# feihoo87/waveforms

Measured on AMD Instinct MI355X. Metric: Msamples/s (all channels), higher is better.
Workload: dtype f64; 1 GPU; sampler256: 256 ch/GPU x 1e+07 pts, 100 gaussian+DRAG pulses/ch, seeds 1000+c (SURVEY 8(d) C4/C5 channel spec), grid mode; channels_per_gpu=256, channels_total=256, points_per_channel=10000000, output=device (HBM) buffer, parallelism=channel-block-per-rank x1, no data-path collective

## Files before the change

### waveforms_amd/csrc/wfk_chain_dev.h

```cpp
#pragma once
#include <hip/hip_runtime.h>

#include <type_traits>
#include <utility>

#include "wfk_internal.h"

namespace {

template <int... K, typename F>
__device__ __forceinline__ void sfor_impl(std::integer_sequence<int, K...>, F&& f) {
  (f(std::integral_constant<int, K>{}), ...);
}
template <int N, typename F>
__device__ __forceinline__ void sfor(F&& f) {
  sfor_impl(std::make_integer_sequence<int, N>{}, static_cast<F&&>(f));
}
#define CH_EACH(N, k) sfor<N>([&](auto k##_) __attribute__((always_inline)) { constexpr int k = decltype(k##_)::value;
#define CH_END });

__device__ __forceinline__ int cuni(int v) { return __builtin_amdgcn_readfirstlane(v); }
__device__ __forceinline__ int64_t cuni64(int64_t v) {
  return (int64_t)(((uint64_t)(uint32_t)cuni((int)(v >> 32)) << 32) | (uint32_t)cuni((int)v));
}

struct ChSeeds { double c, s, g, r; };

__device__ __forceinline__ double kc(double v) {
  asm volatile("" : "+s"(v));
  return v;
}

__device__ __forceinline__ void sincospi_small(double r, double* sn, double* cs) {
  const double a = fabs(r);
  const bool swap = a > 0.25;
  const double z = swap ? 0.5 - a : a;
  const double t = z * 3.141592653589793116 + z * 1.2246467991473532e-16;
  const double t2 = t * t;
  double ps = kc(-2.8114572543455206e-15);
  ps = fma(ps, t2, kc(7.6471637318198164e-13));
  ps = fma(ps, t2, kc(-1.6059043836821613e-10));
  ps = fma(ps, t2, kc(2.5052108385441720e-08));
  ps = fma(ps, t2, kc(-2.7557319223985893e-06));
  ps = fma(ps, t2, kc(1.9841269841269841e-04));
  ps = fma(ps, t2, kc(-8.3333333333333332e-03));
  ps = fma(ps, t2, kc(1.6666666666666666e-01));
  const double s = fma(-t * t2, ps, t);
  double pc = kc(1.5619206968586226e-16);
  pc = fma(pc, t2, kc(-4.7794773323873853e-14));
  pc = fma(pc, t2, kc(1.1470745597729725e-11));
  pc = fma(pc, t2, kc(-2.0876756987868099e-09));
  pc = fma(pc, t2, kc(2.7557319223985888e-07));
  pc = fma(pc, t2, kc(-2.4801587301587302e-05));
  pc = fma(pc, t2, kc(1.3888888888888889e-03));
  pc = fma(pc, t2, kc(-4.1666666666666664e-02));
  pc = fma(pc, t2, kc(0.5));
  const double c = fma(-t2, pc, 1.0);
  const double ss = swap ? c : s, cc = swap ? s : c;
  *sn = r < 0.0 ? -ss : ss;
  *cs = cc;
}

__device__ __forceinline__ double exp_small(double x) {
#pragma clang fp contract(off)
  const double n = rint(x * 1.4426950408889634);
  double r = fma(-n, 6.93147180369123816490e-01, x);
  r = fma(-n, 1.90821492927058770002e-10, r);
  double p = kc(1.1470745597729725e-11);
  p = fma(p, r, kc(1.6059043836821613e-10));
  p = fma(p, r, kc(2.0876756987868099e-09));
  p = fma(p, r, kc(2.5052108385441720e-08));
  p = fma(p, r, kc(2.7557319223985888e-07));
  p = fma(p, r, kc(2.7557319223985893e-06));
  p = fma(p, r, kc(2.4801587301587302e-05));
  p = fma(p, r, kc(1.9841269841269841e-04));
  p = fma(p, r, kc(1.3888888888888889e-03));
  p = fma(p, r, kc(8.3333333333333332e-03));
  p = fma(p, r, kc(4.1666666666666664e-02));
  p = fma(p, r, kc(1.6666666666666666e-01));
  p = fma(p, r, kc(0.5));
  p = fma(p, r, kc(1.0));
  p = fma(p, r, kc(1.0));
  return ldexp(p, (int)n);
}

__device__ __forceinline__ ChSeeds chain_seeds(double theta, double ea, double eb, int carrier, int env) {
#pragma clang fp contract(off)
  ChSeeds o;
  o.c = 1.0; o.s = 0.0; o.g = 1.0; o.r = 1.0;
  if (carrier) {
    const double IPI_HI = 0.31830988618379069, IPI_LO = -1.9678676675182486e-17;
    const double xh = theta * IPI_HI;
    const double xl = fma(theta, IPI_HI, -xh) + theta * IPI_LO;
    const double n = rint(xh);
    double ss, cc;
    sincospi_small((xh - n) + xl, &ss, &cc);
    const bool odd = ((long long)n) & 1;
    o.s = odd ? -ss : ss;
    o.c = odd ? -cc : cc;
  }
  if (env) {
    o.g = exp_small(ea);
    o.r = exp_small(eb);
  }
  return o;
}

template <typename T, int CL, int KC, bool MASK, bool DEG1, bool SEL = false, bool INIT = false>
__device__ __forceinline__ void chain_loop(const double2* tab, const double* r, const ChSeeds& sd, double u0,
                                           double q, T (&acc)[CL], int klo, int khi, ChSeeds& nx) {
  const T c0 = (T)sd.c, s0 = (T)sd.s;
  const T A0 = (T)r[WFK_FCE_A], A1 = (T)r[WFK_FCE_A + 1], A2 = (T)r[WFK_FCE_A + 2], A3 = (T)r[WFK_FCE_A + 3];
  const T B0 = (T)r[WFK_FCE_B], B1 = (T)r[WFK_FCE_B + 1], B2 = (T)r[WFK_FCE_B + 2], B3 = (T)r[WFK_FCE_B + 3];
  const T P0 = DEG1 ? A0 * c0 + B0 * s0 : (T)0, P1 = DEG1 ? A1 * c0 + B1 * s0 : (T)0;
  const T Q0 = DEG1 ? B0 * c0 - A0 * s0 : (T)0, Q1 = DEG1 ? B1 * c0 - A1 * s0 : (T)0;
  double g = sd.g, rr = sd.r;
  T u = (T)u0;
  const T Dt = (T)r[WFK_FCE_D];
#ifndef WFK_FIRS_SB
#define WFK_FIRS_SB 1
#endif
  constexpr int SB = CL % WFK_FIRS_SB == 0 ? WFK_FIRS_SB : 2;
  static_assert(CL % SB == 0, "chain length must be even");
  CH_EACH(CL / SB, kb)
    double2 tb[SB];
    CH_EACH(SB, kk) tb[kk] = tab[kb * SB + kk]; CH_END
    CH_EACH(SB, kk)
      constexpr int k = kb * SB + kk;
      T val;
      if constexpr (DEG1) {
        const T pp = P1 * u + P0, qq = Q1 * u + Q0;
        u += Dt;
        val = (pp * (T)tb[kk].x + qq * (T)tb[kk].y) * (T)g;
      } else {
        const T pa = ((A3 * u + A2) * u + A1) * u + A0;
        const T pb = ((B3 * u + B2) * u + B1) * u + B0;
        u += Dt;
        const T ck = c0 * (T)tb[kk].x - s0 * (T)tb[kk].y;
        const T sk = s0 * (T)tb[kk].x + c0 * (T)tb[kk].y;
        val = (pa * ck + pb * sk) * (T)g;
      }
      if constexpr (k == KC) {
        nx.g = g;
        nx.r = rr;
        nx.c = sd.c * tb[kk].x - sd.s * tb[kk].y;
        nx.s = sd.s * tb[kk].x + sd.c * tb[kk].y;
      }
      g *= rr;
      rr *= q;
      if constexpr (INIT) acc[k] = val;
      else if constexpr (MASK && SEL) acc[k] += (k >= klo && k < khi) ? val : (T)0;
      else if (!MASK || (k >= klo && k < khi)) acc[k] += val;
    CH_END
    __builtin_amdgcn_sched_barrier(0);
  CH_END
  if constexpr (KC == CL) {
    const double2 te = tab[CL];
    nx.g = g;
    nx.r = rr;
    nx.c = sd.c * te.x - sd.s * te.y;
    nx.s = sd.s * te.x + sd.c * te.y;
  }
}

__device__ __forceinline__ ChSeeds chain_make_seeds(const double* r, double x, int fl) {
  const double v = (x - r[WFK_FCE_SG]) / r[WFK_FCE_SIGMA], Hh = r[WFK_FCE_H];
  if (fl & WFK_FCE_EXPENV)
    return chain_seeds(r[WFK_FCE_W] * (x - r[WFK_FCE_SREF]), r[WFK_FCE_SIGMA] * (x - r[WFK_FCE_SG]), Hh,
                       (fl >> 2) & 1, true);
  return chain_seeds(r[WFK_FCE_W] * (x - r[WFK_FCE_SREF]), -(v * v), -Hh * (2.0 * v + Hh), (fl >> 2) & 1,
                     ((fl >> 4) & 3) != 0);
}

template <typename T, int CL, int KC, bool SEL = false>
__device__ __forceinline__ void chain_envmul(const double* r, const ChSeeds& sd, T (&acc)[CL], int klo, int khi,
                                             ChSeeds& nx) {
  double g = sd.g, rr = sd.r;
  const double q = r[WFK_FCE_Q];
  nx = sd;
  CH_EACH(CL, k)
    if constexpr (k == KC) {
      nx.g = g;
      nx.r = rr;
    }
    if constexpr (SEL) acc[k] *= (k >= klo && k < khi) ? (T)g : (T)1;
    else if (k >= klo && k < khi) acc[k] *= (T)g;
    g *= rr;
    rr *= q;
  CH_END
  if constexpr (KC == CL) {
    nx.g = g;
    nx.r = rr;
  }
}

}
```

### waveforms_amd/csrc/wfk_fir_sampled.hip

```cpp
#include <hip/hip_runtime.h>

#include <algorithm>
#include <cmath>
#include <cstring>
#include <memory>
#include <new>
#include <string>
#include <type_traits>
#include <utility>
#include <vector>

#include "wfk.h"
#include "wfk_fft4096.h"
#include "wfk_host.h"
#include "wfk_internal.h"
#include "wfk_short_dev.h"
#include "wfk_chain_dev.h"

namespace {

struct ChainArgs {
  const DevChannel* channels;
  const DevPiece* pieces;
  const double* params;
  const int32_t* pair_first;
  void* out;
  int64_t out_stride, n, npairs;
  const void* hspec;
  const void* tw;
  double t0, step, last;
  int32_t has_last, hop, K, lead;
  int64_t hrow;
  int64_t i0;
};

__device__ __forceinline__ double chain_time(const ChainArgs& a, int64_t j) {
#pragma clang fp contract(off)
  const double m = (double)(j + a.i0) * a.step;
  double t = m + a.t0;
  if (a.has_last && j == a.n - 1) t = a.last;
  return t;
}

#ifndef WFK_FIRS_WAVES
#define WFK_FIRS_WAVES 3
#endif
#ifndef WFK_FIRS_PPW
#define WFK_FIRS_PPW 1
#endif
#define WFK_FIRS_NCAR 2

template <typename T, int HOPB>
__global__ void __launch_bounds__(256, WFK_FIRS_WAVES) fir_sampled(const ChainArgs a) {
  constexpr int CL = 16 + HOPB;
  constexpr int PPW = WFK_FIRS_PPW, NCAR = WFK_FIRS_NCAR;
  constexpr bool CARRY = PPW > 1;
  constexpr int KC = CARRY ? 2 * HOPB : -1;
  static_assert(KC < CL, "the chains of consecutive pairs must overlap");
  __shared__ __attribute__((aligned(16))) T lds[LDS_ELEMS];
  double* const s_par = reinterpret_cast<double*>(lds);
  constexpr int LDS_DOUBLES = (int)(sizeof(T) * LDS_ELEMS / sizeof(double));
  double2* const unit_tab = reinterpret_cast<double2*>(s_par + LDS_DOUBLES - 2 * CL);
  const int tid = threadIdx.x;
  const int ch = blockIdx.y;
  const DevChannel C = a.channels[ch];
  const cx<T>* hspec = static_cast<const cx<T>*>(a.hspec) + (int64_t)ch * a.hrow;
  const cx<T>* tw = static_cast<const cx<T>*>(a.tw);
  T* const orow = static_cast<T*>(a.out) + (int64_t)ch * a.out_stride;
  const int M = a.hop;

  int car_piece = -1;
  ChSeeds car[NCAR];
  for (int i = 0; i < NCAR; ++i) { car[i].c = 1.0; car[i].s = 0.0; car[i].g = 1.0; car[i].r = 1.0; }

  for (int pp = 0; pp < PPW; ++pp) {
    const int64_t pair = (int64_t)blockIdx.x * PPW + pp;
    if (pair >= a.npairs) break;
    const int64_t s1 = 2 * pair * (int64_t)a.hop - a.lead;
    const int64_t range_end = s1 + 256 * (int64_t)CL;

    T acc[CL];
    CH_EACH(CL, k) acc[k] = (T)0; CH_END
    double x = chain_time(a, s1 + tid);
    if (C.tshift != 0.0) x = x - C.tshift;
    __syncthreads();
    if (tid < CL) unit_tab[tid] = make_double2(1.0, 0.0);
    int next_car = -1;
    int q = cuni(a.pair_first[(int64_t)ch * a.npairs + pair]);
    for (; q < C.piece_end; q = cuni(q + 1)) {
      const DevPiece P = a.pieces[q];
      if (P.start >= range_end) break;
      if (P.n_blk == 0 || P.stop <= s1) continue;
      __syncthreads();
      for (int i = tid; i < P.first_len; i += 256) s_par[i] = a.params[P.par_off + i];
      __syncthreads();
      const int nops = cuni((int)s_par[1]);
      const bool full = P.start <= s1 && P.stop >= range_end;
      const bool carried = CARRY && full && car_piece == q;
      int klo = 0, khi = CL;
      if (!full) {
        const int64_t lim = 256 * (int64_t)(CL + 2);
        const int64_t los = P.start - s1, his = P.stop - s1;
        const int lo = (int)(los < -lim ? -lim : (los > lim ? lim : los)) - tid;
        const int hi = (int)(his < -lim ? -lim : (his > lim ? lim : his)) - tid;
        klo = lo <= 0 ? 0 : (lo + 255) >> 8;
        khi = hi <= 0 ? 0 : (hi + 255) >> 8;
        klo = klo > CL ? CL : klo;
        khi = khi > CL ? CL : khi;
      }
      for (int op = 0; op < nops; ++op) {
        const double* rec = s_par + WFK_BLK_HDR + op * WFK_FCE_REC;
        const int fl = cuni(WFK_FCE_WORD(rec));
        const int env = (fl >> 4) & 3, carrier = (fl >> 2) & 1;
        ChSeeds sd, nx;
        if (carried && op == 0) sd = car[0];
        else if (carried && NCAR > 1 && op == 1) sd = car[NCAR > 1 ? 1 : 0];
        else sd = chain_make_seeds(rec, x, fl);
        if (env == 3) {
          chain_envmul<T, CL, KC>(rec, sd, acc, klo, khi, nx);
        } else {
          const double2* tab = carrier ? reinterpret_cast<const double2*>(s_par + WFK_FCE_TABOFF(fl)) : unit_tab;
          const double qq = env ? rec[WFK_FCE_Q] : 1.0;
          const double u0 = x - rec[WFK_FCE_SLIN];
          if (full && (fl & 3) <= 1) chain_loop<T, CL, KC, false, true>(tab, rec, sd, u0, qq, acc, 0, CL, nx);
          else if (full) chain_loop<T, CL, KC, false, false>(tab, rec, sd, u0, qq, acc, 0, CL, nx);
          else chain_loop<T, CL, KC, true, false>(tab, rec, sd, u0, qq, acc, klo, khi, nx);
        }
        if (CARRY && op == 0) car[0] = nx;
        if (CARRY && NCAR > 1 && op == 1) car[NCAR > 1 ? 1 : 0] = nx;
      }
      if (full) next_car = q;
    }
    car_piece = next_car;
    __syncthreads();

    const T base = (T)C.offset;
    const int64_t b1 = 2 * pair, b2 = b1 + 1;
    const bool interior = s1 >= 0 && range_end <= a.n && (b2 + 1) * (int64_t)M <= a.n;
    if (interior) {
      if (base != (T)0) {
        CH_EACH(CL, k) acc[k] += base; CH_END
      }
    } else {
      CH_EACH(CL, k)
        const int64_t j = s1 + tid + 256 * k;
        acc[k] = (j >= 0 && j < a.n) ? acc[k] + base : (T)0;
      CH_END
    }
    cx<T> v[16];
    CH_EACH(16, n1)
      v[n1].x = acc[n1];
      v[n1].y = acc[n1 + HOPB];
    CH_END

    int tf = tid;
    asm volatile("" : "+v"(tf));
    const cx<T> wa = tw[tf], wb = tw[16 * (tf & 15)];
    fft4096<false>(v, lds, wa, wb, tf);
#pragma unroll
    for (int k3 = 0; k3 < 16; ++k3) v[k3] = cmul(v[k3], hspec[tf + 256 * k3]);
    fft4096<true>(v, lds, wa, wb, tf);
    if (interior) {
      T* const o1 = orow + b1 * M + (tf - (a.K - 1));
      T* const o2 = o1 + M;
#pragma unroll
      for (int q3 = 0; q3 < 16; ++q3) {
        const int r = tf + 256 * q3 - (a.K - 1);
        if (r >= 0 && r < M) {
          o1[256 * q3] = v[q3].x;
          o2[256 * q3] = v[q3].y;
        }
      }
    } else {
#pragma unroll
      for (int q3 = 0; q3 < 16; ++q3) {
        const int r = tf + 256 * q3 - (a.K - 1);
        if (r >= 0 && r < M) {
          const int64_t d1 = b1 * M + r, d2 = b2 * M + r;
          if (d1 < a.n) orow[d1] = v[q3].x;
          if (d2 < a.n) orow[d2] = v[q3].y;
        }
      }
    }
  }
}

struct ChainShortArgs {
  const DevChannel* channels;
  const ShortWin* wins;
  const uint32_t* entries;
  const double* recs;
  const void* ws;
  int64_t ws_stride;
  void* out;
  int64_t out_stride, n, npairs;
  const void* hspec;
  const void* tw;
  double step;
  int32_t hop, K, lead;
  int64_t hrow;
};

template <typename T>
__device__ __attribute__((noinline)) void chain_copy_runs(T* lds, const T* wrow, const uint32_t* ents, int ccnt,
                                                          bool sw, int tid) {
  for (int cb = 0; cb < ccnt; cb += 256) {
    const int idx = cb + tid;
    if (idx < ccnt) {
      const uint32_t word = ents[idx];
      const int len = (int)(word >> 28) + 1, o = (int)((word >> 16) & 0xfff);
      T* const b0 = lds + (sw ? o + (o >> 4) : o);
      const int t = sw ? 16 - (o & 15) : 99;
      for (int k = 0; k < len; ++k) *((k >= t ? b0 + 1 : b0) + k) = wrow[o + k];
    }
  }
}

#ifndef WFK_FSH_PARK
#define WFK_FSH_PARK 7
#endif
template <typename T, int HOPB>
__global__ void __launch_bounds__(256, WFK_FIRS_WAVES) fir_short(const ChainShortArgs a) {
  constexpr int CL = 16 + HOPB, HR = CL / 2, HALF = 256 * HR, R = WFK_SH_R;
  static_assert(CL % 2 == 0 && HALF + HALF / 16 <= LDS_ELEMS, "a half window must fit the transform's array");
  static_assert(HALF <= 4096, "entry offsets are 12 bit");
  constexpr int PARK = sizeof(T) == 8 ? WFK_FSH_PARK : 0, PARK_BASE = HALF + HALF / 16;
  constexpr int LDS_ALL = PARK_BASE + 256 * PARK > LDS_ELEMS ? PARK_BASE + 256 * PARK : LDS_ELEMS;
  __shared__ __attribute__((aligned(16))) T lds[LDS_ALL];
  const int tid = threadIdx.x;
  const int ch = blockIdx.y;
  const DevChannel C = a.channels[ch];
  const cx<T>* hspec = static_cast<const cx<T>*>(a.hspec) + (int64_t)ch * a.hrow;
  const cx<T>* tw = static_cast<const cx<T>*>(a.tw);
  T* const orow = static_cast<T*>(a.out) + (int64_t)ch * a.out_stride;
  const int M = a.hop;
  const int64_t pair = blockIdx.x;
  const int64_t s1 = 2 * pair * (int64_t)a.hop - a.lead;
  const int64_t range_end = s1 + 256 * (int64_t)CL;
  const double base = C.offset;

  const ShortWin* const wp0 = a.wins + ((int64_t)ch * a.npairs + pair) * 2;
  int64_t w_rec0[2], w_e0[2];
  int w_cnt[2], w_pad[2], w_ccnt[2];
  uint32_t w_first[2];
  CH_EACH(2, half)
    w_rec0[half] = cuni64(wp0[half].rec0);
    w_e0[half] = cuni64(wp0[half].e0);
    w_cnt[half] = cuni(wp0[half].cnt);
    w_pad[half] = cuni(wp0[half].pad);
    w_ccnt[half] = cuni(wp0[half].ccnt);
    w_first[half] = tid < w_cnt[half] ? a.entries[w_e0[half] + tid] : 0u;
  CH_END


  T x[CL];
  CH_EACH(2, half)
    const int64_t h0 = s1 + (int64_t)HALF * half;
    __syncthreads();
    const bool sw = w_pad[half] != 0;
    T* const mine = lds + (sw ? tid + (tid >> 4) : tid);
    const bool inside = h0 >= 0 && h0 + HALF <= a.n;
    auto prefill = [&](auto rs_) __attribute__((always_inline)) {
      constexpr int rs = decltype(rs_)::value;
      if (inside) {
        CH_EACH(HR, k) mine[rs * k] = (T)base; CH_END
      } else {
        CH_EACH(HR, k)
          const int64_t j = h0 + 256 * k + tid;
          mine[rs * k] = (j >= 0 && j < a.n) ? (T)base : (T)0;
        CH_END
      }
    };
    if (sw) prefill(std::integral_constant<int, 272>{});
    else prefill(std::integral_constant<int, 256>{});
    __syncthreads();
    const int64_t rec0 = w_rec0[half], e0 = w_e0[half];
    const int cnt = w_cnt[half];
    for (int eb = 0; eb < cnt; eb += 256) {
      const int idx = eb + tid;
      bool live = idx < cnt;
      const uint32_t word = eb == 0 ? w_first[half] : (live ? a.entries[e0 + idx] : 0u);
      const int len = live ? (int)(word >> 28) + 1 : 0;
      const int o = (int)((word >> 16) & 0xfff);
      const double* op = a.recs + 2 * (rec0 + (int64_t)(word & 0xffff));
      shdev::OpRec rec = shdev::load_op(op);
      const double kf = (double)((int)(uint32_t)(h0 + o) - shdev::op_ref(rec));
      double acc[R], acci[1];
      CH_EACH(R, k) acc[k] = 0.0; CH_END
      acci[0] = 0.0;
      auto eval = [&](const shdev::OpRec& rc, const double* opp, bool lv) -> bool {
        const int w = shdev::op_word(rc);
        const bool closing = ((w >> 4) & 3) == 3;
        const bool mine = lv && !closing && !(w & 8);
        const bool cubic = __any(mine && (w & 3) > 1);
        if (mine) {
          if (cubic) shdev::short_op<R, true, false>(rc, opp, w, kf, a.step, acc, acci);
          else shdev::short_op<R, false, false>(rc, opp, w, kf, a.step, acc, acci);
        }
        if (__any(lv && closing)) {
          if (lv && closing) shdev::short_erfmul<R, false>(rc, kf, acc, acci);
        }
        return lv && !(w & WFK_SH_LAST);
      };
      live = eval(rec, op, live);
      while (__any(live)) {
        op += (shdev::op_word(rec) & 3) > 1 ? WFK_SH_OP3 : WFK_SH_OP1;
        if (live) rec = shdev::load_op(op);
        live = eval(rec, op, live);
      }
      if (C.do_clip) {
        CH_EACH(R, k) acc[k] = shdev::clip_np(acc[k], C.clip_lo, C.clip_hi); CH_END
      }
      T* const b0 = lds + (sw ? o + (o >> 4) : o);
      const int t = sw ? 16 - (o & 15) : 99;
      CH_EACH(R, k)
        if (k < len) *((k >= t ? b0 + 1 : b0) + k) = (T)(acc[k] + base);
      CH_END
    }
    if (__builtin_expect(w_ccnt[half] != 0, 0))
      chain_copy_runs<T>(lds, static_cast<const T*>(a.ws) + (int64_t)ch * a.ws_stride + h0, a.entries + e0 + cnt,
                         w_ccnt[half], sw, tid);
    __syncthreads();
    auto pickup = [&](auto rs_) __attribute__((always_inline)) {
      constexpr int rs = decltype(rs_)::value;
      CH_EACH(HR, k)
        if constexpr (half == 0 && k >= HR - PARK) lds[PARK_BASE + 256 * (k - (HR - PARK)) + tid] = mine[rs * k];
        else x[half * HR + k] = mine[rs * k];
      CH_END
    };
    if (sw) pickup(std::integral_constant<int, 272>{});
    else pickup(std::integral_constant<int, 256>{});
  CH_END
  CH_EACH(PARK, k) x[HR - PARK + k] = lds[PARK_BASE + 256 * k + tid]; CH_END
  __syncthreads();

  cx<T> v[16];
  CH_EACH(16, n1)
    v[n1].x = x[n1];
    v[n1].y = x[n1 + HOPB];
  CH_END
  const int64_t b1 = 2 * pair, b2 = b1 + 1;
  const bool interior = s1 >= 0 && range_end <= a.n && (b2 + 1) * (int64_t)M <= a.n;

  int tf = tid;
  asm volatile("" : "+v"(tf));
  const cx<T> wa = tw[tf], wb = tw[16 * (tf & 15)];
  fft4096<false>(v, lds, wa, wb, tf);
#pragma unroll
  for (int k3 = 0; k3 < 16; ++k3) v[k3] = cmul(v[k3], hspec[tf + 256 * k3]);
  fft4096<true>(v, lds, wa, wb, tf);
  if (interior) {
    T* const o1 = orow + b1 * M + (tf - (a.K - 1));
    T* const o2 = o1 + M;
#pragma unroll
    for (int q3 = 0; q3 < 16; ++q3) {
      const int r = tf + 256 * q3 - (a.K - 1);
      if (r >= 0 && r < M) {
        o1[256 * q3] = v[q3].x;
        o2[256 * q3] = v[q3].y;
      }
    }
  } else {
#pragma unroll
    for (int q3 = 0; q3 < 16; ++q3) {
      const int r = tf + 256 * q3 - (a.K - 1);
      if (r >= 0 && r < M) {
        const int64_t d1 = b1 * M + r, d2 = b2 * M + r;
        if (d1 < a.n) orow[d1] = v[q3].x;
        if (d2 < a.n) orow[d2] = v[q3].y;
      }
    }
  }
}

}

struct wfk_chain_plan {
  wfk_plan* sampler = nullptr;
  wfk_fir_plan* fir = nullptr;
  bool fused = false;
  int32_t kind = 0, n_channels = 0, hopb = 0;
  int64_t n = 0, npairs = 0;
  std::string why;
  DevBuf<char> d_tables;
  DevChannel* d_channels = nullptr;
  DevPiece* d_pieces = nullptr;
  double* d_params = nullptr;
  int32_t* d_pair_first = nullptr;
  bool shortw = false, hybrid = false;
  ShortWin* d_wins = nullptr;
  uint32_t* d_entries = nullptr;
  const double* d_recs = nullptr;
  int64_t table_bytes = 0;
  double t0 = 0, step = 0, last = 0;
  int32_t has_last = 0;
  int64_t i0 = 0;
  DevBuf<char> workspace;
  ~wfk_chain_plan() {
    if (d_tables || workspace) (void)hipDeviceSynchronize();
    wfk_plan_destroy(sampler);
    wfk_fir_plan_destroy(fir);
  }
};

extern "C" {

int wfk_chain_plan_destroy(wfk_chain_plan* p) {
  delete p;
  return WFK_OK;
}

static int chain_plan_create(const wfk_program* prog, const wfk_grid* grid, const double* ker_host, int32_t K,
                             int kind, wfk_chain_plan** out, bool per_row);

int wfk_chain_plan_create(const wfk_program* prog, const wfk_grid* grid, const double* ker_host, int32_t K,
                          int kind, wfk_chain_plan** out) {
  return chain_plan_create(prog, grid, ker_host, K, kind, out, false);
}

int wfk_chain_plan_create_rows(const wfk_program* prog, const wfk_grid* grid, const double* kers_host, int32_t K,
                               int kind, wfk_chain_plan** out) {
  return chain_plan_create(prog, grid, kers_host, K, kind, out, true);
}

static int chain_plan_create(const wfk_program* prog, const wfk_grid* grid, const double* ker_host, int32_t K,
                             int kind, wfk_chain_plan** out, bool per_row) try {
  if (!out) return wfk_fail(WFK_EINVAL, "null out");
  *out = nullptr;
  if (!prog || !grid || !ker_host) return wfk_fail(WFK_EINVAL, "null argument");
  if (const int rc = wfk_check_kind(kind, "chain ")) return rc;
  std::unique_ptr<wfk_chain_plan> p(new wfk_chain_plan());
  p->kind = kind;
  CompileRequest req;
  req.keep_mixed_short = true;
  int rc = wfk_internal_plan_create(prog, grid, nullptr, 0, req, &p->sampler);
  if (rc) return rc;
  {
    const HostPlan* h0 = nullptr;
    const double* r0 = nullptr;
    wfk_internal_plan_tables(p->sampler, &h0, &r0);
    if (h0 && h0->shortp && h0->short_has_fmul) {
      wfk_plan_destroy(p->sampler);
      p->sampler = nullptr;
      req.no_short_fmul = true;
      rc = wfk_internal_plan_create(prog, grid, nullptr, 0, req, &p->sampler);
      if (rc) return rc;
    }
  }
  p->n = grid->n;
  p->n_channels = prog->n_channels;
  rc = per_row ? wfk_fir_plan_create_rows(ker_host, K, grid->n, std::max(1, prog->n_channels), kind, &p->fir)
               : wfk_fir_plan_create(ker_host, K, grid->n, std::max(1, prog->n_channels), kind, &p->fir);
  if (rc) return rc;
  p->t0 = grid->t0; p->step = grid->step; p->last = grid->last; p->has_last = grid->has_last; p->i0 = grid->i0;
  if (p->n == 0 || p->n_channels == 0) { *out = p.release(); return WFK_OK; }

  const void *kspec = nullptr, *tw = nullptr;
  int fir_fused = 0, nseg = 0, Kf = 0, lead = 0;
  wfk_internal_fir_tables(p->fir, &kspec, &tw, &fir_fused, &nseg, &Kf, &lead);
  const char* off = getenv("WFK_CHAIN_UNFUSED");
  HostPlan H;
  std::string err;
  p->hopb = K <= 1025 ? 12 : 10;
  if (off && off[0] == '1') p->why = "disabled by WFK_CHAIN_UNFUSED";
  else if (!fir_fused || nseg != 1) p->why = "FIR kernel longer than one on-chip transform";
  else if (prog->n_channels > 65535) p->why = "more than 65535 channels";
  else if (wfk_compile_geom(prog, grid, 256, 16 + p->hopb, H, err) != WFK_OK) p->why = "geometry compile: " + err;
  else if (!H.lean) p->why = "plan is not fully fused (generic / direct terms -- erf edges and exponential envelopes included, which this kernel does not evaluate -- or too many ops per piece)";
  else {
    for (const DevChannel& c : H.channels)
      if (c.do_clip) p->why = "clip (min/max) on a channel";
    for (uint8_t cx_ : H.channel_complex)
      if (cx_) p->why = "complex-valued channel";
  }
  if (!p->why.empty() && fir_fused && nseg == 1 && prog->n_channels <= 65535 && !(off && off[0] == '1')) {
    const HostPlan* hs = nullptr;
    const double* d_recs = nullptr;
    wfk_internal_plan_tables(p->sampler, &hs, &d_recs);
    bool real = true;
    if (hs) for (uint8_t cx_ : hs->channel_complex) real = real && !cx_;
    if (hs && d_recs && hs->shortp && real) {
      const int64_t hop = 256 * (int64_t)p->hopb, HALF = 128 * (int64_t)(16 + p->hopb);
      const int64_t nblk = (p->n + hop - 1) / hop;
      p->npairs = (nblk + 1) / 2;
      std::vector<ShortWin> wins;
      std::vector<uint32_t> ents;
      std::string bad;
      (void)wfk_chain_windows(*hs, p->n, hop, lead, HALF, p->npairs, wins, ents, bad);
      if (bad.empty()) {
        if (ents.empty()) ents.push_back(0);
        DevTables t;
        const size_t o_ch = t.add(hs->channels), o_w = t.add(wins), o_e = t.add(ents);
        if (!p->d_tables.alloc(t.total()) || !t.upload(p->d_tables.get()))
          return wfk_fail(WFK_ENOMEM, "chain table allocation failed");
        p->d_channels = t.at<DevChannel>(p->d_tables.get(), o_ch);
        p->d_wins = t.at<ShortWin>(p->d_tables.get(), o_w);
        p->d_entries = t.at<uint32_t>(p->d_tables.get(), o_e);
        p->d_recs = d_recs;
        p->table_bytes = (int64_t)(hs->channels.size() * sizeof(DevChannel) + wins.size() * sizeof(ShortWin) +
                                   ents.size() * sizeof(uint32_t) + hs->params.size() * sizeof(double));
        if (hs->mixed) {
          const size_t es = wfk_elem_size(kind);
          if (!p->workspace.alloc((size_t)p->n_channels * (size_t)p->n * es))
            return wfk_fail(WFK_ENOMEM, "chain workspace allocation failed");
          p->hybrid = true;
        }
        p->shortw = true;
        p->fused = true;
        p->why.clear();
        *out = p.release();
        return WFK_OK;
      }
      p->why += "; short geometry: " + bad;
    }
  }
  if (p->why.empty()) {
    const int64_t hop = 256 * (int64_t)p->hopb;
    const int64_t nblk = (p->n + hop - 1) / hop;
    p->npairs = (nblk + 1) / 2;
    std::vector<int32_t> pair_first((size_t)p->npairs * p->n_channels);
    for (int32_t c = 0; c < p->n_channels; ++c) {
      int32_t q = H.channels[c].piece_begin;
      for (int64_t pr = 0; pr < p->npairs; ++pr) {
        const int64_t s1 = 2 * pr * hop - lead;
        while (q < H.channels[c].piece_end - 1 && H.pieces[q].stop <= s1) ++q;
        pair_first[(size_t)c * p->npairs + pr] = q;
      }
    }
    DevTables t;
    const size_t o_ch = t.add(H.channels), o_pc = t.add(H.pieces), o_pa = t.add(H.params), o_pf = t.add(pair_first);
    if (!p->d_tables.alloc(t.total()) || !t.upload(p->d_tables.get()))
      return wfk_fail(WFK_ENOMEM, "chain table allocation failed");
    p->d_channels = t.at<DevChannel>(p->d_tables.get(), o_ch);
    p->d_pieces = t.at<DevPiece>(p->d_tables.get(), o_pc);
    p->d_params = t.at<double>(p->d_tables.get(), o_pa);
    p->d_pair_first = t.at<int32_t>(p->d_tables.get(), o_pf);
    p->table_bytes = (int64_t)t.total();
    p->fused = true;
  } else {
    const size_t es = wfk_elem_size(kind);
    if (!p->workspace.alloc((size_t)p->n_channels * (size_t)p->n * es))
      return wfk_fail(WFK_ENOMEM, "chain workspace allocation failed");
  }
  *out = p.release();
  return WFK_OK;
} catch (const std::bad_alloc&) {
  return wfk_fail(WFK_ENOMEM, "out of host memory while building the chain plan");
}

int wfk_chain_is_fused(const wfk_chain_plan* p) { return p && p->fused ? 1 : 0; }

const char* wfk_chain_unfused_reason(const wfk_chain_plan* p) { return p ? p->why.c_str() : ""; }

int64_t wfk_chain_table_bytes(const wfk_chain_plan* p) {
  if (!p) return wfk_fail(WFK_EINVAL, "null plan");
  return p->fused ? p->table_bytes : wfk_plan_table_bytes(p->sampler);
}

}

template <typename F>
static auto chain_build(const wfk_chain_plan* p, F&& f) {
  using H12 = std::integral_constant<int, 12>; using H10 = std::integral_constant<int, 10>;
  if (p->kind == WFK_OUT_F32) return p->hopb == 12 ? f(float{}, H12{}) : f(float{}, H10{});
  return p->hopb == 12 ? f(double{}, H12{}) : f(double{}, H10{});
}

extern "C" {

const char* wfk_chain_kernel_name(const wfk_chain_plan* p) {
  if (!p) return "";
  static thread_local std::string name;
  if (p->fused) {
    name = chain_build(p, [&](auto t, auto hop) {
      return std::string(p->shortw ? "fir_short<" : "fir_sampled<") + (sizeof(t) == 4 ? "float" : "double") + "," + std::to_string(hop()) + ">";
    });
    if (p->hybrid) name = "wfk_sample<...> (pieces without a short form) + " + name;
  }
  else name = std::string(wfk_plan_kernel_name(p->sampler, p->kind)) + " + FIR";
  return name.c_str();
}

int wfk_chain_launch(wfk_chain_plan* p, void* out_dev, int64_t out_stride, void* hip_stream) {
  if (!p) return wfk_fail(WFK_EINVAL, "null plan");
  if (p->n == 0 || p->n_channels == 0) return WFK_OK;
  if (const int rc = wfk_check_rows("FIR chain", p->n, wfk_elem_size(p->kind), out_dev, p->n_channels, out_stride,
                                    out_dev, p->n_channels, out_stride))
    return rc;
  hipStream_t s = (hipStream_t)hip_stream;
  if (!p->fused) {
    int rc = wfk_plan_launch(p->sampler, p->workspace.get(), p->n, p->kind, 0, hip_stream);
    if (rc) return rc;
    return wfk_fir_apply(p->fir, p->workspace.get(), p->n, out_dev, out_stride, hip_stream);
  }
  const void *kspec = nullptr, *tw = nullptr;
  int fir_fused = 0, nseg = 0, K = 0, lead = 0;
  wfk_internal_fir_tables(p->fir, &kspec, &tw, &fir_fused, &nseg, &K, &lead);
  if (p->shortw) {
    if (p->hybrid) {
      const int rc = wfk_internal_plan_launch_foreign(p->sampler, p->workspace.get(), p->n, p->kind, hip_stream);
      if (rc) return rc;
    }
    ChainShortArgs a{};
    a.ws = p->workspace.get(); a.ws_stride = p->n;
    a.channels = p->d_channels; a.wins = p->d_wins; a.entries = p->d_entries; a.recs = p->d_recs;
    a.out = out_dev; a.out_stride = out_stride; a.n = p->n; a.npairs = p->npairs;
    a.hspec = kspec; a.tw = tw; a.step = p->step; a.hrow = wfk_internal_fir_krow(p->fir);
    a.hop = 256 * p->hopb; a.K = K; a.lead = lead;
    const dim3 grid((unsigned)p->npairs, (unsigned)p->n_channels);
    chain_build(p, [&](auto t, auto hop) { hipLaunchKernelGGL((fir_short<decltype(t), decltype(hop)::value>), grid, dim3(256), 0, s, a); });
    if (hipGetLastError() != hipSuccess) return wfk_fail(WFK_EHIP, "fused sampler->FIR kernel launch failed");
    return WFK_OK;
  }
  ChainArgs a{};
  a.channels = p->d_channels; a.pieces = p->d_pieces; a.params = p->d_params; a.pair_first = p->d_pair_first;
  a.out = out_dev; a.out_stride = out_stride; a.n = p->n; a.npairs = p->npairs;
  a.hspec = kspec; a.tw = tw; a.hrow = wfk_internal_fir_krow(p->fir);
  a.t0 = p->t0; a.step = p->step; a.last = p->last; a.has_last = p->has_last; a.i0 = p->i0;
  a.hop = 256 * p->hopb; a.K = K; a.lead = lead;
  const dim3 grid((unsigned)((p->npairs + WFK_FIRS_PPW - 1) / WFK_FIRS_PPW), (unsigned)p->n_channels);
  chain_build(p, [&](auto t, auto hop) { hipLaunchKernelGGL((fir_sampled<decltype(t), decltype(hop)::value>), grid, dim3(256), 0, s, a); });
  if (hipGetLastError() != hipSuccess) return wfk_fail(WFK_EHIP, "fused sampler->FIR kernel launch failed");
  return WFK_OK;
}

}
```

Measured before the change: 771,300 Msamples/s.

## Walk several FIR pairs per block with LDS-carried chain seeds and resident params

The fused sampler->FIR kernel now walks a runtime-configurable number of consecutive pairs per block, defaulting to 4 where the old default was 1. Chain seeds carried between pairs now live in LDS rather than registers. Piece parameters are cached in a dedicated LDS buffer and only reloaded when the piece changes, which drops per-piece barriers. Kernel arguments and tables are read through the constant address space via the kernarg pointer to keep values in scalar registers. The aim is to amortise seed recomputation (sincos/exp) and parameter loads across pairs, at the cost of fewer blocks in the grid and more LDS per workgroup, which may limit occupancy.

```diff
diff --git a/waveforms_amd/csrc/wfk_chain_dev.h b/waveforms_amd/csrc/wfk_chain_dev.h
--- a/waveforms_amd/csrc/wfk_chain_dev.h
+++ b/waveforms_amd/csrc/wfk_chain_dev.h
@@ -25,6 +25,19 @@
 }
 
 struct ChSeeds { double c, s, g, r; };
+
+struct ChDrop {
+  __device__ __forceinline__ void operator=(double) const {}
+};
+struct ChSlot {
+  double* p;
+  __device__ __forceinline__ void operator=(double v) const { *p = v; }
+};
+struct ChCarryLds {
+  ChDrop c, s;
+  ChSlot g, r;
+  __device__ __forceinline__ void operator=(const ChSeeds&) const {}
+};
 
 __device__ __forceinline__ double kc(double v) {
   asm volatile("" : "+s"(v));
@@ -106,9 +119,9 @@
   return o;
 }
 
-template <typename T, int CL, int KC, bool MASK, bool DEG1, bool SEL = false, bool INIT = false>
+template <typename T, int CL, int KC, bool MASK, bool DEG1, bool SEL = false, bool INIT = false, typename NX = ChSeeds>
 __device__ __forceinline__ void chain_loop(const double2* tab, const double* r, const ChSeeds& sd, double u0,
-                                           double q, T (&acc)[CL], int klo, int khi, ChSeeds& nx) {
+                                           double q, T (&acc)[CL], int klo, int khi, NX& nx) {
   const T c0 = (T)sd.c, s0 = (T)sd.s;
   const T A0 = (T)r[WFK_FCE_A], A1 = (T)r[WFK_FCE_A + 1], A2 = (T)r[WFK_FCE_A + 2], A3 = (T)r[WFK_FCE_A + 3];
   const T B0 = (T)r[WFK_FCE_B], B1 = (T)r[WFK_FCE_B + 1], B2 = (T)r[WFK_FCE_B + 2], B3 = (T)r[WFK_FCE_B + 3];
@@ -172,9 +185,9 @@
                      ((fl >> 4) & 3) != 0);
 }
 
-template <typename T, int CL, int KC, bool SEL = false>
+template <typename T, int CL, int KC, bool SEL = false, typename NX = ChSeeds>
 __device__ __forceinline__ void chain_envmul(const double* r, const ChSeeds& sd, T (&acc)[CL], int klo, int khi,
-                                             ChSeeds& nx) {
+                                             NX& nx) {
   double g = sd.g, rr = sd.r;
   const double q = r[WFK_FCE_Q];
   nx = sd;
diff --git a/waveforms_amd/csrc/wfk_fir_sampled.hip b/waveforms_amd/csrc/wfk_fir_sampled.hip
--- a/waveforms_amd/csrc/wfk_fir_sampled.hip
+++ b/waveforms_amd/csrc/wfk_fir_sampled.hip
@@ -32,71 +32,121 @@
   int32_t has_last, hop, K, lead;
   int64_t hrow;
   int64_t i0;
+  int32_t ppw;
 };
 
-__device__ __forceinline__ double chain_time(const ChainArgs& a, int64_t j) {
+template <typename Args>
+__device__ __forceinline__ double chain_time(Args a, int64_t j) {
 #pragma clang fp contract(off)
-  const double m = (double)(j + a.i0) * a.step;
-  double t = m + a.t0;
-  if (a.has_last && j == a.n - 1) t = a.last;
+  const double m = (double)(j + a->i0) * a->step;
+  double t = m + a->t0;
+  if (a->has_last && j == a->n - 1) t = a->last;
   return t;
 }
+
+#if defined(__HIP_DEVICE_COMPILE__)
+typedef const __attribute__((address_space(4))) ChainArgs* ChainArgsPtr;
+__device__ __forceinline__ ChainArgsPtr chain_args(const ChainArgs&) {
+  ChainArgsPtr p = (ChainArgsPtr)__builtin_amdgcn_kernarg_segment_ptr();
+  asm volatile("" : "+s"(p));
+  return p;
+}
+#define CH_TABLE(U) const __attribute__((address_space(4))) U*
+template <typename U>
+__device__ __forceinline__ CH_TABLE(U) chain_table(const U* p) {
+  return (CH_TABLE(U))(unsigned long long)p;
+}
+#else
+typedef const ChainArgs* ChainArgsPtr;
+__device__ inline ChainArgsPtr chain_args(const ChainArgs& a) { return &a; }
+#define CH_TABLE(U) const U*
+template <typename U>
+__device__ inline const U* chain_table(const U* p) { return p; }
+#endif
+__device__ __forceinline__ bool ch_lt(int64_t a, int64_t b) { return (int64_t)((uint64_t)a - (uint64_t)b) < 0; }
+struct ChPiece { int64_t start, stop, par_off; int32_t n_blk, first_len; };
 
 #ifndef WFK_FIRS_WAVES
 #define WFK_FIRS_WAVES 3
 #endif
-#ifndef WFK_FIRS_PPW
-#define WFK_FIRS_PPW 1
+#ifndef WFK_FIRS_NCAR
+#define WFK_FIRS_NCAR 1
 #endif
-#define WFK_FIRS_NCAR 2
+#ifndef WFK_FIRS_RES
+#define WFK_FIRS_RES 504
+#endif
+#define WFK_FIRS_PPW_MAX 5
+#ifndef WFK_FIRS_PPW_DEFAULT
+#define WFK_FIRS_PPW_DEFAULT 4
+#endif
 
 template <typename T, int HOPB>
-__global__ void __launch_bounds__(256, WFK_FIRS_WAVES) fir_sampled(const ChainArgs a) {
+__global__ void __launch_bounds__(256, WFK_FIRS_WAVES) fir_sampled(const ChainArgs a_) {
   constexpr int CL = 16 + HOPB;
-  constexpr int PPW = WFK_FIRS_PPW, NCAR = WFK_FIRS_NCAR;
-  constexpr bool CARRY = PPW > 1;
-  constexpr int KC = CARRY ? 2 * HOPB : -1;
+  constexpr int NCAR = WFK_FIRS_NCAR, RES = WFK_FIRS_RES;
+  constexpr int KC = 2 * HOPB;
   static_assert(KC < CL, "the chains of consecutive pairs must overlap");
+  static_assert(2 * HOPB * (WFK_FIRS_PPW_MAX - 1) + CL <= 128, "a walk must stay inside the reseed interval the suite holds");
   __shared__ __attribute__((aligned(16))) T lds[LDS_ELEMS];
-  double* const s_par = reinterpret_cast<double*>(lds);
-  constexpr int LDS_DOUBLES = (int)(sizeof(T) * LDS_ELEMS / sizeof(double));
-  double2* const unit_tab = reinterpret_cast<double2*>(s_par + LDS_DOUBLES - 2 * CL);
-  const int tid = threadIdx.x;
-  const int ch = blockIdx.y;
-  const DevChannel C = a.channels[ch];
-  const cx<T>* hspec = static_cast<const cx<T>*>(a.hspec) + (int64_t)ch * a.hrow;
-  const cx<T>* tw = static_cast<const cx<T>*>(a.tw);
-  T* const orow = static_cast<T*>(a.out) + (int64_t)ch * a.out_stride;
-  const int M = a.hop;
+  __shared__ __attribute__((aligned(16))) double s_res[RES];
+  __shared__ __attribute__((aligned(16))) double2 unit_tab[CL];
+  __shared__ double s_car[(NCAR * 4 + 2) * 256];
+  static_assert(3 * (sizeof(T) * LDS_ELEMS + sizeof(double) * (RES + 2 * CL + (NCAR * 4 + 2) * 256)) <= 160 * 1024,
+                "three workgroups per CU");
+  double* const s_arr = reinterpret_cast<double*>(lds);
 
   int car_piece = -1;
-  ChSeeds car[NCAR];
-  for (int i = 0; i < NCAR; ++i) { car[i].c = 1.0; car[i].s = 0.0; car[i].g = 1.0; car[i].r = 1.0; }
-
-  for (int pp = 0; pp < PPW; ++pp) {
-    const int64_t pair = (int64_t)blockIdx.x * PPW + pp;
-    if (pair >= a.npairs) break;
-    const int64_t s1 = 2 * pair * (int64_t)a.hop - a.lead;
+  int res_piece = -1;
+  if (threadIdx.x < CL) unit_tab[threadIdx.x] = make_double2(1.0, 0.0);
+
+  int tid = threadIdx.x;
+  for (int pp = 0;; ++pp) {
+    const ChainArgsPtr a = chain_args(a_);
+    int ch = blockIdx.y;
+    asm volatile("" : "+v"(tid));
+    asm volatile("" : "+s"(ch));
+    const int ppw = a->ppw;
+    const int64_t pair = (int64_t)blockIdx.x * ppw + pp;
+    if (pp >= ppw || pair >= a->npairs) break;
+    CH_TABLE(DevChannel) const cp = chain_table(a->channels) + ch;
+    struct { double offset, tshift; int32_t piece_end; } C = {cp->offset, cp->tshift, cp->piece_end};
+    const cx<T>* hspec = static_cast<const cx<T>*>(a->hspec) + (int64_t)ch * a->hrow;
+    const cx<T>* tw = static_cast<const cx<T>*>(a->tw);
+    T* const orow = static_cast<T*>(a->out) + (int64_t)ch * a->out_stride;
+    const int M = a->hop;
+    const int64_t s1 = 2 * pair * (int64_t)a->hop - a->lead;
     const int64_t range_end = s1 + 256 * (int64_t)CL;
+    const bool more = pp + 1 < ppw && pair + 1 < a->npairs;
+    const bool last_row = a->has_last && a->n - 1 >= s1 && a->n - 1 < s1 + 256;
 
     T acc[CL];
     CH_EACH(CL, k) acc[k] = (T)0; CH_END
     double x = chain_time(a, s1 + tid);
     if (C.tshift != 0.0) x = x - C.tshift;
-    __syncthreads();
-    if (tid < CL) unit_tab[tid] = make_double2(1.0, 0.0);
     int next_car = -1;
-    int q = cuni(a.pair_first[(int64_t)ch * a.npairs + pair]);
+    bool in_array = false;
+    int q = cuni(chain_table(a->pair_first)[(int64_t)ch * a->npairs + pair]);
     for (; q < C.piece_end; q = cuni(q + 1)) {
-      const DevPiece P = a.pieces[q];
-      if (P.start >= range_end) break;
-      if (P.n_blk == 0 || P.stop <= s1) continue;
-      __syncthreads();
-      for (int i = tid; i < P.first_len; i += 256) s_par[i] = a.params[P.par_off + i];
-      __syncthreads();
+      CH_TABLE(DevPiece) const pq = chain_table(a->pieces) + q;
+      const ChPiece P = {pq->start, pq->stop, pq->par_off, pq->n_blk, pq->first_len};
+      if (!ch_lt(P.start, range_end)) break;
+      if (P.n_blk == 0 || !ch_lt(s1, P.stop)) continue;
+      const int blen = cuni(P.first_len);
+      const bool fits = blen <= RES;
+      const double* const s_par = fits ? s_res : s_arr;
+      if (!fits || res_piece != q) {
+        __syncthreads();
+        double* const dst = fits ? s_res : s_arr;
+        int i0 = tid;
+        asm volatile("" : "+v"(i0));
+        for (int i = i0; i < blen; i += 256) dst[i] = a->params[P.par_off + i];
+        __syncthreads();
+        if (fits) res_piece = q;
+        else in_array = true;
+      }
       const int nops = cuni((int)s_par[1]);
-      const bool full = P.start <= s1 && P.stop >= range_end;
-      const bool carried = CARRY && full && car_piece == q;
+      const bool full = !ch_lt(s1, P.start) && !ch_lt(P.stop, range_end);
+      const bool carried = full && car_piece == q && !last_row;
       int klo = 0, khi = CL;
       if (!full) {
         const int64_t lim = 256 * (int64_t)(CL + 2);
@@ -112,31 +162,49 @@
         const double* rec = s_par + WFK_BLK_HDR + op * WFK_FCE_REC;
         const int fl = cuni(WFK_FCE_WORD(rec));
         const int env = (fl >> 4) & 3, carrier = (fl >> 2) & 1;
-        ChSeeds sd, nx;
-        if (carried && op == 0) sd = car[0];
-        else if (carried && NCAR > 1 && op == 1) sd = car[NCAR > 1 ? 1 : 0];
-        else sd = chain_make_seeds(rec, x, fl);
+        double* const mine = s_car + (op < NCAR ? op * 4 : NCAR * 4 - 2) * 256 + tid;
+        ChSeeds sd;
+        if (carried && op < NCAR) {
+          sd.c = mine[0]; sd.s = mine[256]; sd.g = mine[512]; sd.r = mine[768];
+        } else {
+          sd = chain_make_seeds(rec, x, fl);
+        }
+        const bool hand_on = more && full && op < NCAR;
+        ChCarryLds nx;
+        nx.g.p = mine + 512;
+        nx.r.p = mine + 768;
         if (env == 3) {
-          chain_envmul<T, CL, KC>(rec, sd, acc, klo, khi, nx);
+          if (hand_on) { mine[0] = sd.c; mine[256] = sd.s; }
+          int kl = klo, kh = khi;
+          asm volatile("" : "+v"(kl), "+v"(kh));
+          chain_envmul<T, CL, KC>(rec, sd, acc, kl, kh, nx);
         } else {
           const double2* tab = carrier ? reinterpret_cast<const double2*>(s_par + WFK_FCE_TABOFF(fl)) : unit_tab;
+          if (hand_on) {
+            const double2 te = tab[KC];
+            mine[0] = sd.c * te.x - sd.s * te.y;
+            mine[256] = sd.s * te.x + sd.c * te.y;
+          }
           const double qq = env ? rec[WFK_FCE_Q] : 1.0;
           const double u0 = x - rec[WFK_FCE_SLIN];
           if (full && (fl & 3) <= 1) chain_loop<T, CL, KC, false, true>(tab, rec, sd, u0, qq, acc, 0, CL, nx);
           else if (full) chain_loop<T, CL, KC, false, false>(tab, rec, sd, u0, qq, acc, 0, CL, nx);
-          else chain_loop<T, CL, KC, true, false>(tab, rec, sd, u0, qq, acc, klo, khi, nx);
+          else {
+            int kl = klo, kh = khi;
+            asm volatile("" : "+v"(kl), "+v"(kh));
+            chain_loop<T, CL, KC, true, false>(tab, rec, sd, u0, qq, acc, kl, kh, nx);
+          }
         }
-        if (CARRY && op == 0) car[0] = nx;
-        if (CARRY && NCAR > 1 && op == 1) car[NCAR > 1 ? 1 : 0] = nx;
       }
       if (full) next_car = q;
     }
     car_piece = next_car;
-    __syncthreads();
+    if (in_array) __syncthreads();
+    asm volatile("" : "+v"(tid));
 
     const T base = (T)C.offset;
     const int64_t b1 = 2 * pair, b2 = b1 + 1;
-    const bool interior = s1 >= 0 && range_end <= a.n && (b2 + 1) * (int64_t)M <= a.n;
+    const bool interior = s1 >= 0 && range_end <= a->n && (b2 + 1) * (int64_t)M <= a->n;
     if (interior) {
       if (base != (T)0) {
         CH_EACH(CL, k) acc[k] += base; CH_END
@@ -144,7 +212,7 @@
     } else {
       CH_EACH(CL, k)
         const int64_t j = s1 + tid + 256 * k;
-        acc[k] = (j >= 0 && j < a.n) ? acc[k] + base : (T)0;
+        acc[k] = (j >= 0 && j < a->n) ? acc[k] + base : (T)0;
       CH_END
     }
     cx<T> v[16];
@@ -153,19 +221,19 @@
       v[n1].y = acc[n1 + HOPB];
     CH_END
 
-    int tf = tid;
-    asm volatile("" : "+v"(tf));
+    asm volatile("" : "+v"(tid));
+    const int tf = tid;
     const cx<T> wa = tw[tf], wb = tw[16 * (tf & 15)];
     fft4096<false>(v, lds, wa, wb, tf);
 #pragma unroll
     for (int k3 = 0; k3 < 16; ++k3) v[k3] = cmul(v[k3], hspec[tf + 256 * k3]);
     fft4096<true>(v, lds, wa, wb, tf);
     if (interior) {
-      T* const o1 = orow + b1 * M + (tf - (a.K - 1));
+      T* const o1 = orow + b1 * M + (tf - (a->K - 1));
       T* const o2 = o1 + M;
 #pragma unroll
       for (int q3 = 0; q3 < 16; ++q3) {
-        const int r = tf + 256 * q3 - (a.K - 1);
+        const int r = tf + 256 * q3 - (a->K - 1);
         if (r >= 0 && r < M) {
           o1[256 * q3] = v[q3].x;
           o2[256 * q3] = v[q3].y;
@@ -174,11 +242,11 @@
     } else {
 #pragma unroll
       for (int q3 = 0; q3 < 16; ++q3) {
-        const int r = tf + 256 * q3 - (a.K - 1);
+        const int r = tf + 256 * q3 - (a->K - 1);
         if (r >= 0 && r < M) {
           const int64_t d1 = b1 * M + r, d2 = b2 * M + r;
-          if (d1 < a.n) orow[d1] = v[q3].x;
-          if (d2 < a.n) orow[d2] = v[q3].y;
+          if (d1 < a->n) orow[d1] = v[q3].x;
+          if (d2 < a->n) orow[d2] = v[q3].y;
         }
       }
     }
@@ -380,6 +448,7 @@
   wfk_fir_plan* fir = nullptr;
   bool fused = false;
   int32_t kind = 0, n_channels = 0, hopb = 0;
+  int32_t ppw = WFK_FIRS_PPW_DEFAULT;
   int64_t n = 0, npairs = 0;
   std::string why;
   DevBuf<char> d_tables;
@@ -459,6 +528,8 @@
   int fir_fused = 0, nseg = 0, Kf = 0, lead = 0;
   wfk_internal_fir_tables(p->fir, &kspec, &tw, &fir_fused, &nseg, &Kf, &lead);
   const char* off = getenv("WFK_CHAIN_UNFUSED");
+  if (const char* w = getenv("WFK_FIRS_PPW"))
+    if (w[0] >= '1' && w[0] <= '0' + WFK_FIRS_PPW_MAX && !w[1]) p->ppw = w[0] - '0';
   HostPlan H;
   std::string err;
   p->hopb = K <= 1025 ? 12 : 10;
@@ -617,8 +688,8 @@
   a.out = out_dev; a.out_stride = out_stride; a.n = p->n; a.npairs = p->npairs;
   a.hspec = kspec; a.tw = tw; a.hrow = wfk_internal_fir_krow(p->fir);
   a.t0 = p->t0; a.step = p->step; a.last = p->last; a.has_last = p->has_last; a.i0 = p->i0;
-  a.hop = 256 * p->hopb; a.K = K; a.lead = lead;
-  const dim3 grid((unsigned)((p->npairs + WFK_FIRS_PPW - 1) / WFK_FIRS_PPW), (unsigned)p->n_channels);
+  a.hop = 256 * p->hopb; a.K = K; a.lead = lead; a.ppw = p->ppw;
+  const dim3 grid((unsigned)((p->npairs + p->ppw - 1) / p->ppw), (unsigned)p->n_channels);
   chain_build(p, [&](auto t, auto hop) { hipLaunchKernelGGL((fir_sampled<decltype(t), decltype(hop)::value>), grid, dim3(256), 0, s, a); });
   if (hipGetLastError() != hipSuccess) return wfk_fail(WFK_EHIP, "fused sampler->FIR kernel launch failed");
   return WFK_OK;
```

Result: slower. 742,100 Msamples/s (-3.8%).
